# bjg-gh/style_transfer_visualizer

Hardware: AMD Instinct MI355X
Metric: optimization steps/sec at 512² and 1024², 1/2/4/8 MI355X (higher is better)
Workload: dtype bf16; 1 GPU; single 512x512 image per GPU, L-BFGS (max_iter=1, history 100), VGG19 bf16 storage / fp32 accumulate, fp32 Gram, --no-video (BASELINE.json configs[1]); weights: synthetic He-scaled; size=512, images=1, init_method=random, parallelism=replicas x1 (independent images), lbfgs_history_prefill_steps=95, world_size=1

## Files before the change

### style_transfer_visualizer_amd/csrc/gram.hip

```cpp
#include <stdlib.h>

#include "stv_common.h"

namespace {

constexpr int PK = 32;

template <int TS>
struct GramCfg {
  static constexpr int AT = TS / 64;
  static constexpr int PITCH = TS + 4;
  static constexpr int TILE_FLOATS = PK * PITCH;
  static constexpr int STAGE_FLOATS = 2 * TILE_FLOATS;
  static constexpr int LDS_BYTES = 2 * STAGE_FLOATS * 4;
};

inline int gram_tile(int C) { return C <= 64 ? 64 : 128; }

__device__ __forceinline__ uint32_t split_word(float f) {
  const uint32_t hb = (uint32_t)f32_to_bf16(f);
  const float hf = __uint_as_float(hb << 16);
  const float r = __builtin_isfinite(hf) ? f - hf : 0.0f;
  return hb | ((uint32_t)f32_to_bf16(r) << 16);
}

template <typename T, int TS, bool X3 = false>
__device__ __forceinline__ void gram_partial_body(const T* __restrict__ F, float* __restrict__ partials, int N, int C,
                                                  int ksplit, int chunk, int bx, int by) {
  using G = GramCfg<TS>;
  constexpr int kVec = elem_traits<T>::kVec;
  constexpr int VPR = TS / kVec;
  constexpr int VECS = PK * VPR;
  constexpr int ITERS = (VECS + 255) / 256;
  extern __shared__ __attribute__((aligned(16))) char smem_raw[];
  float* smem = reinterpret_cast<float*>(smem_raw);

  const int nt = (C + TS - 1) / TS;
  int ti = 0, rem = bx;
  while (rem >= nt - ti) { rem -= nt - ti; ++ti; }
  const int tj = ti + rem;
  const int i0 = ti * TS, j0 = tj * TS;
  const int ks = by;
  const int p_begin = ks * chunk;
  const int p_end = min(N, p_begin + chunk);

  const int tid = threadIdx.x, lane = tid & 63, wave = tid >> 6;
  const int wi = wave >> 1, wj = wave & 1;
  const int r = lane & 31, h = lane >> 5;

  f32x16 acc[G::AT][G::AT];
#pragma unroll
  for (int a = 0; a < G::AT; ++a)
#pragma unroll
    for (int b = 0; b < G::AT; ++b)
#pragma unroll
      for (int i = 0; i < 16; ++i) acc[a][b][i] = 0.0f;

  u32x4 reg_i[ITERS], reg_j[ITERS];
  const u32x4 zero4 = {0u, 0u, 0u, 0u};
  auto stage_load = [&](int p0) {
#pragma unroll
    for (int it = 0; it < ITERS; ++it) {
      const int v = it * 256 + tid;
      const int p = p0 + v / VPR, cv = (v % VPR) * kVec;
      const bool okp = (v < VECS) && p < p_end;
      reg_i[it] = (okp && i0 + cv < C) ? *reinterpret_cast<const u32x4*>(F + (size_t)p * C + i0 + cv) : zero4;
      reg_j[it] = (okp && j0 + cv < C) ? *reinterpret_cast<const u32x4*>(F + (size_t)p * C + j0 + cv) : zero4;
    }
  };
  auto stage_write = [&](float* buf) {
#pragma unroll
    for (int it = 0; it < ITERS; ++it) {
      const int v = it * 256 + tid;
      if (v < VECS) {
        const int pr = v / VPR, cv = (v % VPR) * kVec;
        float fi[kVec], fj[kVec];
        unpack16<T>(reg_i[it], fi);
        unpack16<T>(reg_j[it], fj);
        if constexpr (X3) {
#pragma unroll
          for (int e = 0; e < kVec; ++e) {
            fi[e] = __uint_as_float(split_word(fi[e]));
            fj[e] = __uint_as_float(split_word(fj[e]));
          }
        }
#pragma unroll
        for (int q = 0; q < kVec / 4; ++q) {
          *reinterpret_cast<f32x4*>(buf + pr * G::PITCH + cv + 4 * q) =
              f32x4{fi[4 * q], fi[4 * q + 1], fi[4 * q + 2], fi[4 * q + 3]};
          *reinterpret_cast<f32x4*>(buf + G::TILE_FLOATS + pr * G::PITCH + cv + 4 * q) =
              f32x4{fj[4 * q], fj[4 * q + 1], fj[4 * q + 2], fj[4 * q + 3]};
        }
      }
    }
  };

  const int nstages = (p_end > p_begin) ? (p_end - p_begin + PK - 1) / PK : 0;
  if (nstages > 0) {
    stage_load(p_begin);
    stage_write(smem);
  }
  __syncthreads();
  for (int s = 0; s < nstages; ++s) {
    float* cur = smem + (s & 1) * G::STAGE_FLOATS;
    float* nxt = smem + ((s + 1) & 1) * G::STAGE_FLOATS;
    const bool more = (s + 1) < nstages;
    if (more) stage_load(p_begin + (s + 1) * PK);
    const float* ai = cur + wi * (G::AT * 32) + r;
    const float* bj = cur + G::TILE_FLOATS + wj * (G::AT * 32) + r;
    if constexpr (X3) {
      auto frag = [&](const float* base, bf16x8v& hi, bf16x8v& lo) {
        uint32_t w[8];
#pragma unroll
        for (int e = 0; e < 8; ++e) w[e] = __float_as_uint(base[(8 * h + e) * G::PITCH]);
        u32x4 vh, vl;
#pragma unroll
        for (int e = 0; e < 4; ++e) {
          vh[e] = __builtin_amdgcn_perm(w[2 * e + 1], w[2 * e], 0x05040100u);
          vl[e] = __builtin_amdgcn_perm(w[2 * e + 1], w[2 * e], 0x07060302u);
        }
        hi = __builtin_bit_cast(bf16x8v, vh);
        lo = __builtin_bit_cast(bf16x8v, vl);
      };
#pragma unroll
      for (int kk = 0; kk < PK / 16; ++kk) {
        bf16x8v ah[G::AT], al[G::AT], bh[G::AT], bl[G::AT];
#pragma unroll
        for (int a = 0; a < G::AT; ++a) frag(ai + kk * 16 * G::PITCH + a * 32, ah[a], al[a]);
#pragma unroll
        for (int b = 0; b < G::AT; ++b) frag(bj + kk * 16 * G::PITCH + b * 32, bh[b], bl[b]);
#pragma unroll
        for (int a = 0; a < G::AT; ++a)
#pragma unroll
          for (int b = 0; b < G::AT; ++b) {
            acc[a][b] = __builtin_amdgcn_mfma_f32_32x32x16_bf16(ah[a], bh[b], acc[a][b], 0, 0, 0);
            acc[a][b] = __builtin_amdgcn_mfma_f32_32x32x16_bf16(ah[a], bl[b], acc[a][b], 0, 0, 0);
            acc[a][b] = __builtin_amdgcn_mfma_f32_32x32x16_bf16(al[a], bh[b], acc[a][b], 0, 0, 0);
          }
      }
    } else
#pragma unroll
    for (int q = 0; q < PK / 2; ++q) {
      float av[G::AT], bv[G::AT];
#pragma unroll
      for (int a = 0; a < G::AT; ++a) av[a] = ai[(2 * q + h) * G::PITCH + a * 32];
#pragma unroll
      for (int b = 0; b < G::AT; ++b) bv[b] = bj[(2 * q + h) * G::PITCH + b * 32];
#pragma unroll
      for (int a = 0; a < G::AT; ++a)
#pragma unroll
        for (int b = 0; b < G::AT; ++b)
          acc[a][b] = __builtin_amdgcn_mfma_f32_32x32x2f32(av[a], bv[b], acc[a][b], 0, 0, 0);
    }
    if (more) stage_write(nxt);
    __syncthreads();
  }

  float* out = partials + (size_t)ks * C * C;
#pragma unroll
  for (int a = 0; a < G::AT; ++a)
#pragma unroll
    for (int b = 0; b < G::AT; ++b)
#pragma unroll
      for (int i = 0; i < 16; ++i) {
        const int row = i0 + wi * (G::AT * 32) + a * 32 + (i & 3) + 8 * (i >> 2) + 4 * h;
        const int col = j0 + wj * (G::AT * 32) + b * 32 + r;
        if (row < C && col < C) out[(size_t)row * C + col] = acc[a][b][i];
      }
}

constexpr int kMaxTaps = 8;
struct PartialMulti {
  int n;
  int block0[kMaxTaps + 1];
  const void* F[kMaxTaps];
  float* partials[kMaxTaps];
  int N[kMaxTaps], C[kMaxTaps], ksplit[kMaxTaps], chunk[kMaxTaps], pairs[kMaxTaps];
};
__device__ __forceinline__ int find_tap(const int* block0, int n, int b) {
  int i = 0;
  while (i + 1 < n && b >= block0[i + 1]) ++i;
  return i;
}

__device__ __forceinline__ void decode_block(int b, int pairs, int ksplit, int& pair, int& ks) {
  pair = b % pairs;
  ks = b / pairs;
}

using PartialSingleFn = void (*)(const void*, float*, int, int, int, int, int);
template <typename T, int TS, bool X3 = false>
__global__ __launch_bounds__(256) void gram_partial_kernel(const void* __restrict__ F, float* __restrict__ partials,
                                                           int N, int C, int ksplit, int chunk, int pairs) {
  int pair, ks;
  decode_block(blockIdx.x, pairs, ksplit, pair, ks);
  gram_partial_body<T, TS, X3>(static_cast<const T*>(F), partials, N, C, ksplit, chunk, pair, ks);
}
template <typename T, int TS, bool X3 = false>
__global__ __launch_bounds__(256) void gram_partial_multi_kernel(PartialMulti m) {
  const int i = find_tap(m.block0, m.n, blockIdx.x);
  const int b = blockIdx.x - m.block0[i];
  int pair, ks;
  decode_block(b, m.pairs[i], m.ksplit[i], pair, ks);
  gram_partial_body<T, TS, X3>(static_cast<const T*>(m.F[i]), m.partials[i], m.N[i], m.C[i], m.ksplit[i], m.chunk[i],
                           pair, ks);
}

typedef __attribute__((ext_vector_type(4))) short s16x4;
typedef __attribute__((address_space(3))) s16x4 lds_s16x4;

#ifndef STV_GRAM_PKB
#define STV_GRAM_PKB 64
#endif
constexpr int PKB = STV_GRAM_PKB;

template <int TS>
struct GramBCfg {
  static constexpr int AT = TS / 64;
  static constexpr int PITCH = TS * 2 + 64;
  static constexpr int TILE_BYTES = PKB * PITCH;
  static constexpr int STAGE_BYTES = 2 * TILE_BYTES;
  static constexpr int LDS_BYTES = 2 * STAGE_BYTES;
};

#ifdef STV_GRAM_STAMPS
__device__ unsigned long long g_gram_stamps[8];
#define GRAM_T() wall_clock64()
#else
#define GRAM_T() 0ull
#endif

template <int TS>
__device__ __forceinline__ void gram_partial_bf16_body(const bf16_t* __restrict__ F, float* __restrict__ partials,
                                                       int N, int C, int ksplit, int chunk, int bx, int by) {
  using G = GramBCfg<TS>;
  constexpr int VPR = TS / 8;
  constexpr int VECS = PKB * VPR;
  constexpr int ITERS = VECS / 256;
  static_assert(VECS % 256 == 0, "whole iterations");
  extern __shared__ __attribute__((aligned(16))) char smem[];

  const int nt = (C + TS - 1) / TS;
  int ti = 0, rem = bx;
  while (rem >= nt - ti) { rem -= nt - ti; ++ti; }
  const int tj = ti + rem;
  const bool same = ti == tj;
  const int i0 = ti * TS, j0 = tj * TS;
  const int ks = by;
  const int p_begin = ks * chunk;
  const int p_end = min(N, p_begin + chunk);

  const int tid = threadIdx.x, lane = tid & 63, wave = tid >> 6;
  const int wi = wave >> 1, wj = wave & 1;
  const int grp = lane >> 4, lam = lane & 15;
  const int tr_lane = ((grp >> 1) * 8 + (lam >> 2)) * G::PITCH + ((grp & 1) * 16 + (lam & 3) * 4) * 2;

  f32x16 acc[G::AT][G::AT];
#pragma unroll
  for (int a = 0; a < G::AT; ++a)
#pragma unroll
    for (int b = 0; b < G::AT; ++b)
#pragma unroll
      for (int i = 0; i < 16; ++i) acc[a][b][i] = 0.0f;

  const __amdgpu_buffer_rsrc_t rs = __builtin_amdgcn_make_buffer_rsrc(
      const_cast<bf16_t*>(F), 0, N * C * 2, 0x00020000);
  const __amdgpu_buffer_rsrc_t rs_null = __builtin_amdgcn_make_buffer_rsrc(const_cast<bf16_t*>(F), 0, 0, 0x00020000);
  constexpr uint32_t kOob = 0x80000000u;
  uint32_t off_i[ITERS], off_j[ITERS];
  int lds_off[ITERS];
#pragma unroll
  for (int it = 0; it < ITERS; ++it) {
    const int v = it * 256 + tid;
    const int pr = v / VPR, cv = (v % VPR) * 8;
    lds_off[it] = pr * G::PITCH + cv * 2;
    off_i[it] = (i0 + cv < C) ? (uint32_t)((pr * C + i0 + cv) * 2) : kOob;
    off_j[it] = (j0 + cv < C) ? (uint32_t)((pr * C + j0 + cv) * 2) : kOob;
  }
  u32x4 reg_i[ITERS], reg_j[ITERS];
  auto stage_load = [&](int p0, bool live) {
    const int rows = min(PKB, p_end - p0);
    const __amdgpu_buffer_rsrc_t r =
        (live && rows > 0) ? __builtin_amdgcn_make_buffer_rsrc(const_cast<bf16_t*>(F) + (size_t)p0 * C, 0,
                                                               rows * C * 2, 0x00020000)
                           : rs_null;
#pragma unroll
    for (int it = 0; it < ITERS; ++it) {
      reg_i[it] = __builtin_amdgcn_raw_buffer_load_b128(r, off_i[it], 0, 0);
      if (!same) reg_j[it] = __builtin_amdgcn_raw_buffer_load_b128(r, off_j[it], 0, 0);
    }
  };
  auto stage_write = [&](char* buf) {
#pragma unroll
    for (int it = 0; it < ITERS; ++it) {
      *reinterpret_cast<u32x4*>(buf + lds_off[it]) = reg_i[it];
      if (!same) *reinterpret_cast<u32x4*>(buf + G::TILE_BYTES + lds_off[it]) = reg_j[it];
    }
  };
  (void)rs;

  const int nstages = (p_end > p_begin) ? (p_end - p_begin + PKB - 1) / PKB : 0;
  unsigned long long tt[6] = {0, 0, 0, 0, 0, 0};
  const unsigned long long t_begin = GRAM_T();
  stage_load(p_begin, nstages > 0);
  stage_write(smem);
  __syncthreads();
  const unsigned long long t_loop = GRAM_T();
  for (int s = 0; s < nstages; ++s) {
    const unsigned long long t0 = GRAM_T();
    char* cur = smem + (s & 1) * G::STAGE_BYTES;
    char* nxt = smem + ((s + 1) & 1) * G::STAGE_BYTES;
    stage_load(p_begin + (s + 1) * PKB, (s + 1) < nstages);
    __builtin_amdgcn_sched_barrier(0);
    const char* ta = cur + tr_lane + (wi * (G::AT * 32)) * 2;
    const char* tb = cur + (same ? 0 : G::TILE_BYTES) + tr_lane + (wj * (G::AT * 32)) * 2;
#pragma unroll
    for (int kk = 0; kk < PKB / 16; ++kk) {
      bf16x8v af[G::AT], bfr[G::AT];
#pragma unroll
      for (int a = 0; a < G::AT; ++a) {
        const char* pa = ta + kk * 16 * G::PITCH + a * 64;
        const s16x4 lo = __builtin_amdgcn_ds_read_tr16_b64_v4i16((lds_s16x4*)(pa));
        const s16x4 hi = __builtin_amdgcn_ds_read_tr16_b64_v4i16((lds_s16x4*)(pa + 4 * G::PITCH));
        typedef __attribute__((ext_vector_type(8))) short s16x8;
        const s16x8 v = {lo[0], lo[1], lo[2], lo[3], hi[0], hi[1], hi[2], hi[3]};
        af[a] = __builtin_bit_cast(bf16x8v, v);
      }
#pragma unroll
      for (int b = 0; b < G::AT; ++b) {
        const char* pb = tb + kk * 16 * G::PITCH + b * 64;
        const s16x4 lo = __builtin_amdgcn_ds_read_tr16_b64_v4i16((lds_s16x4*)(pb));
        const s16x4 hi = __builtin_amdgcn_ds_read_tr16_b64_v4i16((lds_s16x4*)(pb + 4 * G::PITCH));
        typedef __attribute__((ext_vector_type(8))) short s16x8;
        const s16x8 v = {lo[0], lo[1], lo[2], lo[3], hi[0], hi[1], hi[2], hi[3]};
        bfr[b] = __builtin_bit_cast(bf16x8v, v);
      }
#pragma unroll
      for (int a = 0; a < G::AT; ++a)
#pragma unroll
        for (int b = 0; b < G::AT; ++b)
          acc[a][b] = __builtin_amdgcn_mfma_f32_32x32x16_bf16(af[a], bfr[b], acc[a][b], 0, 0, 0);
    }
    __builtin_amdgcn_sched_barrier(0);
#ifdef STV_GRAM_STAMPS
    const unsigned long long t1 = GRAM_T();
    __builtin_amdgcn_s_waitcnt(0x0F70);
    const unsigned long long t2 = GRAM_T();
    stage_write(nxt);
    __builtin_amdgcn_s_waitcnt(0xC07F);
    const unsigned long long t3 = GRAM_T();
    __syncthreads();
    const unsigned long long t4 = GRAM_T();
    tt[0] += t1 - t0; tt[1] += t2 - t1; tt[2] += t3 - t2; tt[3] += t4 - t3;
#else
    stage_write(nxt);
    __syncthreads();
#endif
  }
  const unsigned long long t_end = GRAM_T();

  const int r = lane & 31, h = lane >> 5;
  float* out = partials + (size_t)ks * C * C;
#pragma unroll
  for (int a = 0; a < G::AT; ++a)
#pragma unroll
    for (int b = 0; b < G::AT; ++b)
#pragma unroll
      for (int i = 0; i < 16; ++i) {
        const int row = i0 + wi * (G::AT * 32) + a * 32 + (i & 3) + 8 * (i >> 2) + 4 * h;
        const int col = j0 + wj * (G::AT * 32) + b * 32 + r;
        if (row < C && col < C) out[(size_t)row * C + col] = acc[a][b][i];
      }
#ifdef STV_GRAM_STAMPS
  if (bx == 0 && by == 0 && tid == 0) {
    g_gram_stamps[0] = tt[0]; g_gram_stamps[1] = tt[1]; g_gram_stamps[2] = tt[2]; g_gram_stamps[3] = tt[3];
    g_gram_stamps[4] = t_loop - t_begin; g_gram_stamps[5] = GRAM_T() - t_end; g_gram_stamps[6] = nstages;
  }
#endif
}

template <int TS>
__global__ __launch_bounds__(256) void gram_partial_bf16_kernel(const void* __restrict__ F, float* __restrict__ partials,
                                                                int N, int C, int ksplit, int chunk, int pairs) {
  int pair, ks;
  decode_block(blockIdx.x, pairs, ksplit, pair, ks);
  gram_partial_bf16_body<TS>(static_cast<const bf16_t*>(F), partials, N, C, ksplit, chunk, pair, ks);
}
template <int TS>
__global__ __launch_bounds__(256) void gram_partial_bf16_multi_kernel(PartialMulti m) {
  const int i = find_tap(m.block0, m.n, blockIdx.x);
  const int b = blockIdx.x - m.block0[i];
  int pair, ks;
  decode_block(b, m.pairs[i], m.ksplit[i], pair, ks);
  gram_partial_bf16_body<TS>(static_cast<const bf16_t*>(m.F[i]), m.partials[i], m.N[i], m.C[i], m.ksplit[i],
                             m.chunk[i], pair, ks);
}

__global__ __launch_bounds__(256) void gram_partial_bf16_both_kernel(PartialMulti m128, PartialMulti m64) {
  const int n128 = m128.block0[m128.n];
  int pair, ks;
  if ((int)blockIdx.x < n128) {
    const int i = find_tap(m128.block0, m128.n, blockIdx.x);
    decode_block(blockIdx.x - m128.block0[i], m128.pairs[i], m128.ksplit[i], pair, ks);
    gram_partial_bf16_body<128>(static_cast<const bf16_t*>(m128.F[i]), m128.partials[i], m128.N[i], m128.C[i],
                                m128.ksplit[i], m128.chunk[i], pair, ks);
  } else {
    const int b = (int)blockIdx.x - n128;
    const int i = find_tap(m64.block0, m64.n, b);
    decode_block(b - m64.block0[i], m64.pairs[i], m64.ksplit[i], pair, ks);
    gram_partial_bf16_body<64>(static_cast<const bf16_t*>(m64.F[i]), m64.partials[i], m64.N[i], m64.C[i], m64.ksplit[i],
                               m64.chunk[i], pair, ks);
  }
}

constexpr int FIN_V = 4, FIN_L = 32, FIN_E = FIN_L * FIN_V, FIN_U = 4;
template <typename T, int FIN_S>
__device__ __forceinline__ void gram_finish_body(
    const float* __restrict__ partials, const float* __restrict__ target, float* __restrict__ gram_out,
    float* __restrict__ loss_part, T* __restrict__ sgrad, int C, int TS, int ksplit, float clamp_max,
    float norm, float k_grad, const float* __restrict__ coef_dev, int bx) {
  __shared__ f32x4 red[FIN_S][FIN_L];
  const int le = threadIdx.x % FIN_L;
  const int slice = threadIdx.x / FIN_L;
  const int e = bx * FIN_E + le * FIN_V;
  const int CC = C * C;
  const int i = e / C, j = e - i * C;
  const bool lower = (i / TS) > (j / TS);
  const bool mirror = (i / TS) < (j / TS);
  const f32x4 zero = {0.f, 0.f, 0.f, 0.f};
  f32x4 s = zero;
  if (e < CC && !lower) {
    f32x4 acc[FIN_U];
#pragma unroll
    for (int u = 0; u < FIN_U; ++u) acc[u] = zero;
    const float* src = partials + e;
    int ks = slice;
    for (; ks + (FIN_U - 1) * FIN_S < ksplit; ks += FIN_U * FIN_S) {
#pragma unroll
      for (int u = 0; u < FIN_U; ++u)
        acc[u] += *reinterpret_cast<const f32x4*>(src + (size_t)(ks + u * FIN_S) * CC);
    }
#pragma unroll
    for (int u = 0; u < FIN_U; ++u)
      if (ks + u * FIN_S < ksplit) acc[u] += *reinterpret_cast<const f32x4*>(src + (size_t)(ks + u * FIN_S) * CC);
    s = (acc[0] + acc[1]) + (acc[2] + acc[3]);
  }
  red[slice][le] = s;
  __syncthreads();
  if (slice == 0) {
    float d2 = 0.0f;
    if (e < CC && !lower) {
      f32x4 R = zero;
#pragma unroll
      for (int q = 0; q < FIN_S; ++q) R += red[q][le];
      const float kk = (target && sgrad) ? k_grad * (coef_dev ? *coef_dev : 1.0f) : 0.0f;
      f32x4 Gv, tv = zero;
#pragma unroll
      for (int v = 0; v < FIN_V; ++v) Gv[v] = fminf(R[v], clamp_max) / norm;
      if (gram_out) *reinterpret_cast<f32x4*>(gram_out + e) = Gv;
      if (target) {
        tv = *reinterpret_cast<const f32x4*>(target + e);
#pragma unroll
        for (int v = 0; v < FIN_V; ++v) {
          const float d = Gv[v] - tv[v];
          d2 += d * d;
          if (sgrad) elem_traits<T>::store(sgrad + e + v, (R[v] <= clamp_max) ? kk * d : 0.0f);
        }
      }
      if (mirror) {
#pragma unroll
        for (int v = 0; v < FIN_V; ++v) {
          const int em = (j + v) * C + i;
          if (gram_out) gram_out[em] = Gv[v];
          if (target) {
            const float dm = Gv[v] - target[em];
            d2 += dm * dm;
            if (sgrad) elem_traits<T>::store(sgrad + em, (R[v] <= clamp_max) ? kk * dm : 0.0f);
          }
        }
      }
    }
#pragma unroll
    for (int o = FIN_L / 2; o > 0; o >>= 1) d2 += __shfl_xor(d2, o, FIN_L);
    if (le == 0 && loss_part) loss_part[bx] = d2;
  }
}

struct FinishMulti {
  int n;
  int block0[kMaxTaps + 1];
  const float* partials[kMaxTaps];
  const float* target[kMaxTaps];
  float* gram_out[kMaxTaps];
  float* loss_part[kMaxTaps];
  void* sgrad[kMaxTaps];
  const float* coef_dev[kMaxTaps];
  int C[kMaxTaps], TS[kMaxTaps], ksplit[kMaxTaps];
  float clamp_max[kMaxTaps], norm[kMaxTaps], k_grad[kMaxTaps];
};
template <typename T, int FIN_S>
__global__ __launch_bounds__(FIN_L * FIN_S) void gram_finish_multi_kernel(FinishMulti m) {
  const int i = find_tap(m.block0, m.n, blockIdx.x);
  gram_finish_body<T, FIN_S>(m.partials[i], m.target[i], m.gram_out[i], m.loss_part[i], static_cast<T*>(m.sgrad[i]), m.C[i],
                         m.TS[i], m.ksplit[i], m.clamp_max[i], m.norm[i], m.k_grad[i], m.coef_dev[i],
                         blockIdx.x - m.block0[i]);
}

void add_tap(PartialMulti& m, const void* F, float* partials, int N, int C, int pk) {
  const int nt = ceil_div(C, gram_tile(C)), pairs = nt * (nt + 1) / 2;
  const int ksplit = stv_gram_ksplit(N, C);
  const int k = m.n++;
  m.F[k] = F; m.partials[k] = partials; m.N[k] = N; m.C[k] = C;
  m.ksplit[k] = ksplit; m.chunk[k] = ceil_div(ceil_div(N, ksplit), pk) * pk; m.pairs[k] = pairs;
  m.block0[k + 1] = m.block0[k] + pairs * ksplit;
}

enum { BODY_F32 = STV_F32, BODY_BF16 = STV_BF16, BODY_X3 = STV_BF16X3, BODY_BF16_WIDE };
static_assert(BODY_F32 == 0 && BODY_BF16 == 1 && BODY_X3 == 2, "the table below is indexed by dtype code");
struct PartialKernel {
  PartialSingleFn single;
  void (*multi)(PartialMulti);
  int lds;
};
#define STV_GENERIC(T, X3, TS) {gram_partial_kernel<T, TS, X3>, gram_partial_multi_kernel<T, TS, X3>, GramCfg<TS>::LDS_BYTES}
const PartialKernel kPartialKernels[4][2] = {
    {STV_GENERIC(float, false, 64), STV_GENERIC(float, false, 128)},
    {{gram_partial_bf16_kernel<64>, gram_partial_bf16_multi_kernel<64>, GramBCfg<64>::LDS_BYTES},
     {gram_partial_bf16_kernel<128>, gram_partial_bf16_multi_kernel<128>, GramBCfg<128>::LDS_BYTES}},
    {STV_GENERIC(float, true, 64), STV_GENERIC(float, true, 128)},
    {{gram_partial_kernel<bf16_t, 64>, nullptr, GramCfg<64>::LDS_BYTES}, {gram_partial_kernel<bf16_t, 128>, nullptr, GramCfg<128>::LDS_BYTES}},
};
#undef STV_GENERIC
constexpr int kBothLds = GramBCfg<128>::LDS_BYTES > GramBCfg<64>::LDS_BYTES ? GramBCfg<128>::LDS_BYTES : GramBCfg<64>::LDS_BYTES;

inline int pixels_per_stage(int body) { return body == BODY_BF16 ? PKB : PK; }

int launch_partial(int body, int TS, const PartialMulti& m, hipStream_t st) {
  const PartialKernel& k = kPartialKernels[body][TS == 128];
  const dim3 grid(m.block0[m.n]), block(256);
  if (m.n == 1) {
    if (stv_set_max_lds(reinterpret_cast<const void*>(k.single), k.lds) != STV_OK) return STV_ERR_LAUNCH;
    hipLaunchKernelGGL(k.single, grid, block, k.lds, st, m.F[0], m.partials[0], m.N[0], m.C[0], m.ksplit[0], m.chunk[0], m.pairs[0]);
  } else {
    if (!k.multi) return STV_ERR_ARG;
    if (stv_set_max_lds(reinterpret_cast<const void*>(k.multi), k.lds) != STV_OK) return STV_ERR_LAUNCH;
    hipLaunchKernelGGL(k.multi, grid, block, k.lds, st, m);
  }
  STV_CHECK_LAUNCH();
  return STV_OK;
}

void add_finish_tap(FinishMulti& f, const stv_gram_tap_t& t) {
  const int k = f.n++;
  f.partials[k] = t.partials; f.target[k] = t.target; f.gram_out[k] = t.gram_out; f.loss_part[k] = t.loss_part;
  f.sgrad[k] = t.sgrad; f.coef_dev[k] = t.coef_dev; f.C[k] = t.channels; f.TS[k] = gram_tile(t.channels);
  f.ksplit[k] = stv_gram_ksplit(t.n_pixels, t.channels);
  f.clamp_max[k] = t.clamp_max; f.norm[k] = t.norm;
  f.k_grad[k] = t.coef * 4.0f / ((float)t.channels * (float)t.channels * t.norm);
  f.block0[k + 1] = f.block0[k] + stv_gram_loss_parts(t.channels);
}

template <typename T, int S>
int launch_finish_as(const FinishMulti& f, hipStream_t st) {
  hipLaunchKernelGGL((gram_finish_multi_kernel<T, S>), dim3(f.block0[f.n]), dim3(FIN_L * S), 0, st, f);
  STV_CHECK_LAUNCH();
  return STV_OK;
}
int launch_finish(const FinishMulti& f, bool bf16_seed, bool deep, hipStream_t st) {
  if (bf16_seed) return deep ? launch_finish_as<bf16_t, 32>(f, st) : launch_finish_as<bf16_t, 8>(f, st);
  return deep ? launch_finish_as<float, 32>(f, st) : launch_finish_as<float, 8>(f, st);
}

}

extern "C" int stv_gram_ksplit(int n_pixels, int channels) {
  const int TS = gram_tile(channels);
  const int nt = ceil_div(channels, TS);
  const int pairs = nt * (nt + 1) / 2;
  static const int wg_max = getenv("STV_GRAM_WGS") ? atoi(getenv("STV_GRAM_WGS")) : 512;
  static const int wg_min = getenv("STV_GRAM_WGS_MIN") ? atoi(getenv("STV_GRAM_WGS_MIN")) : 128;
  const int lo = ceil_div(wg_min, pairs), hi = (wg_max / pairs) > 0 ? wg_max / pairs : 1;
  static const int kdiv = getenv("STV_GRAM_KDIV") ? atoi(getenv("STV_GRAM_KDIV")) : 8;
  int ks = n_pixels / (kdiv * channels);
  if (ks < lo) ks = lo;
  if (ks > hi) ks = hi;
  const int max_ks = ceil_div(n_pixels, 64);
  if (ks > max_ks) ks = max_ks;
  if (ks < 1) ks = 1;
  return ks;
}

extern "C" size_t stv_gram_partials_bytes(int n_pixels, int channels) {
  return (size_t)stv_gram_ksplit(n_pixels, channels) * channels * channels * sizeof(float);
}

extern "C" int stv_gram_loss_parts(int channels) { return ceil_div(channels * channels, FIN_E); }

extern "C" int stv_gram_partial(const void* F, float* partials, int n_pixels, int C, int dtype,
                                void* stream) {
  if (!F || !partials || n_pixels <= 0 || C <= 0) return STV_ERR_ARG;
  if (dtype != STV_F32 && dtype != STV_BF16 && dtype != STV_BF16X3) return STV_ERR_ARG;
  const bool bf16 = dtype == STV_BF16;
  if (C % (bf16 ? 8 : 4)) return STV_ERR_ARG;
  const bool huge = (size_t)n_pixels * C * (bf16 ? 2 : 4) >= ((size_t)1 << 31);
  if (dtype == STV_BF16X3 && huge) return STV_ERR_ARG;
  const int body = (bf16 && huge) ? BODY_BF16_WIDE : dtype;
  PartialMulti m{};
  add_tap(m, F, partials, n_pixels, C, pixels_per_stage(body));
  return launch_partial(body, gram_tile(C), m, static_cast<hipStream_t>(stream));
}

extern "C" int stv_gram_finish(const float* partials, const float* target, float* gram_out,
                               float* loss_part, void* sgrad, int n_pixels, int C, float clamp_max,
                               float norm, float coef, const float* coef_dev, int dtype, void* stream) {
  if (!partials || n_pixels <= 0 || C <= 0 || norm <= 0.0f) return STV_ERR_ARG;
  if (dtype != STV_F32 && dtype != STV_BF16) return STV_ERR_ARG;
  FinishMulti f{};
  add_finish_tap(f, stv_gram_tap_t{nullptr, const_cast<float*>(partials), target, gram_out, loss_part, sgrad, coef_dev,
                                   n_pixels, C, clamp_max, norm, coef});
  return launch_finish(f, dtype == STV_BF16, f.ksplit[0] >= 128, static_cast<hipStream_t>(stream));
}

extern "C" int stv_gram_multi(const stv_gram_tap_t* taps, int n_taps, int dtype, void* stream) {
  if (!taps || n_taps <= 0 || n_taps > kMaxTaps) return STV_ERR_ARG;
  if (dtype != STV_F32 && dtype != STV_BF16 && dtype != STV_BF16X3) return STV_ERR_ARG;
  hipStream_t st = static_cast<hipStream_t>(stream);
  const bool x3 = dtype == STV_BF16X3;
  const int vec = dtype == STV_BF16 ? 8 : 4;
  for (int i = 0; i < n_taps; ++i) {
    const stv_gram_tap_t& t = taps[i];
    if (!t.partials || t.n_pixels <= 0 || t.channels <= 0 || t.channels % vec || t.norm <= 0.0f) return STV_ERR_ARG;
    if (dtype == STV_BF16 && (size_t)t.n_pixels * t.channels * 2 >= ((size_t)1 << 31)) return STV_ERR_ARG;
    if (x3 && t.F && (size_t)t.n_pixels * t.channels * 4 >= ((size_t)1 << 31)) return STV_ERR_ARG;
  }
  PartialMulti by_tile[2] = {};
  for (int i = 0; i < n_taps; ++i) {
    const stv_gram_tap_t& t = taps[i];
    if (!t.F) continue;
    add_tap(by_tile[gram_tile(t.channels) == 128], t.F, t.partials, t.n_pixels, t.channels, pixels_per_stage(dtype));
  }
  const PartialMulti& m64 = by_tile[0];
  const PartialMulti& m128 = by_tile[1];
  if (dtype == STV_BF16 && m64.n && m128.n) {
    if (stv_set_max_lds(reinterpret_cast<const void*>(&gram_partial_bf16_both_kernel), kBothLds) != STV_OK) return STV_ERR_LAUNCH;
    hipLaunchKernelGGL(gram_partial_bf16_both_kernel, dim3(m128.block0[m128.n] + m64.block0[m64.n]), dim3(256), kBothLds, st,
                       m128, m64);
    STV_CHECK_LAUNCH();
  } else {
    for (int TS : {64, 128}) {
      const PartialMulti& m = by_tile[TS == 128];
      if (!m.n) continue;
      if (const int rc = launch_partial(dtype, TS, m, st)) return rc;
    }
  }
  FinishMulti f{};
  for (int i = 0; i < n_taps; ++i) add_finish_tap(f, taps[i]);
  return launch_finish(f, dtype == STV_BF16, false, st);
}

#ifdef STV_GRAM_STAMPS
extern "C" int stv_debug_gram_stamps(unsigned long long* out8) {
  return hipMemcpyFromSymbol(out8, HIP_SYMBOL(g_gram_stamps), sizeof(g_gram_stamps)) == hipSuccess ? 0 : 1;
}
#endif
```

Measured before the change: 1248 steps/s.

## Split gram finish into short and long paths with batched partial loads

```diff
diff --git a/style_transfer_visualizer_amd/csrc/gram.hip b/style_transfer_visualizer_amd/csrc/gram.hip
--- a/style_transfer_visualizer_amd/csrc/gram.hip
+++ b/style_transfer_visualizer_amd/csrc/gram.hip
@@ -414,74 +414,196 @@
 }
 
 constexpr int FIN_V = 4, FIN_L = 32, FIN_E = FIN_L * FIN_V, FIN_U = 4;
+constexpr int FIN_HOIST = 4;
+
+inline int finish_blocks(int C, int ksplit, int fin_s) {
+  const int parts = ceil_div(C * C, FIN_E);
+  return ksplit <= FIN_U * fin_s ? ceil_div(parts, fin_s) : parts;
+}
+
+struct FinishQuad {
+  int e, i, j;
+  bool live, mirror;
+};
+__device__ __forceinline__ FinishQuad finish_quad(int e, int C, int TS) {
+  FinishQuad q;
+  q.e = e;
+  q.i = e / C;
+  q.j = e - q.i * C;
+  q.live = e < C * C && (q.i / TS) <= (q.j / TS);
+  q.mirror = (q.i / TS) < (q.j / TS);
+  return q;
+}
+
+struct FinishTargets {
+  f32x4 own;
+  float mir[FIN_V];
+  float coef;
+};
+__device__ __forceinline__ FinishTargets finish_request_targets(const float* __restrict__ target,
+                                                                const float* __restrict__ coef_dev, const FinishQuad& q, int C) {
+  FinishTargets t;
+  t.coef = coef_dev ? *coef_dev : 1.0f;
+  t.own = f32x4{0.f, 0.f, 0.f, 0.f};
+#pragma unroll
+  for (int v = 0; v < FIN_V; ++v) t.mir[v] = 0.0f;
+  if (target) {
+    t.own = *reinterpret_cast<const f32x4*>(target + q.e);
+    if (q.mirror) {
+#pragma unroll
+      for (int v = 0; v < FIN_V; ++v) t.mir[v] = target[(q.j + v) * C + q.i];
+    }
+  }
+  return t;
+}
+
+template <typename T>
+__device__ __forceinline__ float finish_store(const f32x4 R, const FinishTargets& t, const FinishQuad& q,
+                                              const float* __restrict__ target, float* __restrict__ gram_out,
+                                              T* __restrict__ sgrad, int C, float clamp_max, float norm, float k_grad) {
+  float d2 = 0.0f;
+  const float kk = (target && sgrad) ? k_grad * t.coef : 0.0f;
+  f32x4 Gv;
+#pragma unroll
+  for (int v = 0; v < FIN_V; ++v) Gv[v] = fminf(R[v], clamp_max) / norm;
+  if (gram_out) *reinterpret_cast<f32x4*>(gram_out + q.e) = Gv;
+  if (target) {
+    float d[FIN_V];
+#pragma unroll
+    for (int v = 0; v < FIN_V; ++v) d[v] = Gv[v] - t.own[v];
+    static_assert(FIN_V == 4, "the chain below");
+    d2 = fmaf(d[3], d[3], fmaf(d[2], d[2], fmaf(d[0], d[0], d[1] * d[1])));
+    if (sgrad) {
+#pragma unroll
+      for (int v = 0; v < FIN_V; ++v) elem_traits<T>::store(sgrad + q.e + v, (R[v] <= clamp_max) ? kk * d[v] : 0.0f);
+    }
+  }
+  if (q.mirror) {
+#pragma unroll
+    for (int v = 0; v < FIN_V; ++v) {
+      const int em = (q.j + v) * C + q.i;
+      if (gram_out) gram_out[em] = Gv[v];
+      if (target) {
+        const float dm = Gv[v] - t.mir[v];
+        d2 = fmaf(dm, dm, d2);
+        if (sgrad) elem_traits<T>::store(sgrad + em, (R[v] <= clamp_max) ? kk * dm : 0.0f);
+      }
+    }
+  }
+  return d2;
+}
+
+__device__ __forceinline__ float finish_group_sum(float d2) {
+#pragma unroll
+  for (int o = FIN_L / 2; o > 0; o >>= 1) d2 += __shfl_xor(d2, o, FIN_L);
+  return d2;
+}
+
 template <typename T, int FIN_S>
-__device__ __forceinline__ void gram_finish_body(
+__device__ __forceinline__ void gram_finish_short(
+    const float* __restrict__ partials, const float* __restrict__ target, float* __restrict__ gram_out,
+    float* __restrict__ loss_part, T* __restrict__ sgrad, int C, int TS, int ksplit, float clamp_max,
+    float norm, float k_grad, const float* __restrict__ coef_dev, int bx) {
+  constexpr int B = FIN_S <= 8 ? FIN_S : 4;
+  static_assert(FIN_S % B == 0, "whole batches");
+  const int le = threadIdx.x % FIN_L;
+  const int grp = bx * FIN_S + threadIdx.x / FIN_L;
+  const int CC = C * C;
+  const FinishQuad q = finish_quad(grp * FIN_E + le * FIN_V, C, TS);
+  const f32x4 zero = {0.f, 0.f, 0.f, 0.f};
+  float d2 = 0.0f;
+  if (q.live) {
+    const float* src = partials + q.e;
+    f32x4 val[B][FIN_U];
+    auto request = [&](int q0) {
+#pragma unroll
+      for (int b = 0; b < B; ++b)
+#pragma unroll
+        for (int u = 0; u < FIN_U; ++u) {
+          const int ks = q0 + b + u * FIN_S;
+          val[b][u] = ks < ksplit ? *reinterpret_cast<const f32x4*>(src + (size_t)ks * CC) : zero;
+        }
+    };
+    const FinishTargets t = finish_request_targets(target, coef_dev, q, C);
+    f32x4 R = zero;
+#pragma unroll 1
+    for (int q0 = 0; q0 < FIN_S; q0 += B) {
+      request(q0);
+#pragma unroll
+      for (int b = 0; b < B; ++b)
+#pragma unroll
+        for (int u = 0; u < FIN_U; ++u) asm volatile("" : "+v"(val[b][u]));
+#pragma unroll
+      for (int b = 0; b < B; ++b) {
+        f32x4 acc[FIN_U];
+#pragma unroll
+        for (int u = 0; u < FIN_U; ++u) acc[u] = zero + val[b][u];
+        R += (acc[0] + acc[1]) + (acc[2] + acc[3]);
+      }
+    }
+    d2 = finish_store<T>(R, t, q, target, gram_out, sgrad, C, clamp_max, norm, k_grad);
+  }
+  d2 = finish_group_sum(d2);
+  if (le == 0 && loss_part && grp * FIN_E < CC) loss_part[grp] = d2;
+}
+
+template <typename T, int FIN_S>
+__device__ __forceinline__ void gram_finish_long(
     const float* __restrict__ partials, const float* __restrict__ target, float* __restrict__ gram_out,
     float* __restrict__ loss_part, T* __restrict__ sgrad, int C, int TS, int ksplit, float clamp_max,
     float norm, float k_grad, const float* __restrict__ coef_dev, int bx) {
   __shared__ f32x4 red[FIN_S][FIN_L];
   const int le = threadIdx.x % FIN_L;
   const int slice = threadIdx.x / FIN_L;
-  const int e = bx * FIN_E + le * FIN_V;
   const int CC = C * C;
-  const int i = e / C, j = e - i * C;
-  const bool lower = (i / TS) > (j / TS);
-  const bool mirror = (i / TS) < (j / TS);
+  const FinishQuad q = finish_quad(bx * FIN_E + le * FIN_V, C, TS);
   const f32x4 zero = {0.f, 0.f, 0.f, 0.f};
   f32x4 s = zero;
-  if (e < CC && !lower) {
+  FinishTargets t{};
+  if (slice == 0 && q.live) t = finish_request_targets(target, coef_dev, q, C);
+  if (q.live) {
     f32x4 acc[FIN_U];
 #pragma unroll
     for (int u = 0; u < FIN_U; ++u) acc[u] = zero;
-    const float* src = partials + e;
+    const float* src = partials + q.e;
+    f32x4 val[FIN_HOIST][FIN_U];
     int ks = slice;
-    for (; ks + (FIN_U - 1) * FIN_S < ksplit; ks += FIN_U * FIN_S) {
+    for (; ks + (FIN_HOIST * FIN_U - 1) * FIN_S < ksplit; ks += FIN_HOIST * FIN_U * FIN_S) {
+#pragma unroll
+      for (int h = 0; h < FIN_HOIST; ++h)
+#pragma unroll
+        for (int u = 0; u < FIN_U; ++u)
+          val[h][u] = *reinterpret_cast<const f32x4*>(src + (size_t)(ks + (h * FIN_U + u) * FIN_S) * CC);
+#pragma unroll
+      for (int h = 0; h < FIN_HOIST; ++h)
+#pragma unroll
+        for (int u = 0; u < FIN_U; ++u) acc[u] += val[h][u];
+    }
+#pragma unroll
+    for (int h = 0; h < FIN_HOIST; ++h)
+#pragma unroll
+      for (int u = 0; u < FIN_U; ++u) {
+        const int k = ks + (h * FIN_U + u) * FIN_S;
+        if (k < ksplit) val[h][u] = *reinterpret_cast<const f32x4*>(src + (size_t)k * CC);
+      }
+#pragma unroll
+    for (int h = 0; h < FIN_HOIST; ++h)
 #pragma unroll
       for (int u = 0; u < FIN_U; ++u)
-        acc[u] += *reinterpret_cast<const f32x4*>(src + (size_t)(ks + u * FIN_S) * CC);
-    }
-#pragma unroll
-    for (int u = 0; u < FIN_U; ++u)
-      if (ks + u * FIN_S < ksplit) acc[u] += *reinterpret_cast<const f32x4*>(src + (size_t)(ks + u * FIN_S) * CC);
+        if (ks + (h * FIN_U + u) * FIN_S < ksplit) acc[u] += val[h][u];
     s = (acc[0] + acc[1]) + (acc[2] + acc[3]);
   }
   red[slice][le] = s;
   __syncthreads();
   if (slice == 0) {
     float d2 = 0.0f;
-    if (e < CC && !lower) {
+    if (q.live) {
       f32x4 R = zero;
 #pragma unroll
-      for (int q = 0; q < FIN_S; ++q) R += red[q][le];
-      const float kk = (target && sgrad) ? k_grad * (coef_dev ? *coef_dev : 1.0f) : 0.0f;
-      f32x4 Gv, tv = zero;
-#pragma unroll
-      for (int v = 0; v < FIN_V; ++v) Gv[v] = fminf(R[v], clamp_max) / norm;
-      if (gram_out) *reinterpret_cast<f32x4*>(gram_out + e) = Gv;
-      if (target) {
-        tv = *reinterpret_cast<const f32x4*>(target + e);
-#pragma unroll
-        for (int v = 0; v < FIN_V; ++v) {
-          const float d = Gv[v] - tv[v];
-          d2 += d * d;
-          if (sgrad) elem_traits<T>::store(sgrad + e + v, (R[v] <= clamp_max) ? kk * d : 0.0f);
-        }
-      }
-      if (mirror) {
-#pragma unroll
-        for (int v = 0; v < FIN_V; ++v) {
-          const int em = (j + v) * C + i;
-          if (gram_out) gram_out[em] = Gv[v];
-          if (target) {
-            const float dm = Gv[v] - target[em];
-            d2 += dm * dm;
-            if (sgrad) elem_traits<T>::store(sgrad + em, (R[v] <= clamp_max) ? kk * dm : 0.0f);
-          }
-        }
-      }
-    }
-#pragma unroll
-    for (int o = FIN_L / 2; o > 0; o >>= 1) d2 += __shfl_xor(d2, o, FIN_L);
+      for (int k = 0; k < FIN_S; ++k) R += red[k][le];
+      d2 = finish_store<T>(R, t, q, target, gram_out, sgrad, C, clamp_max, norm, k_grad);
+    }
+    d2 = finish_group_sum(d2);
     if (le == 0 && loss_part) loss_part[bx] = d2;
   }
 }
@@ -501,9 +623,13 @@
 template <typename T, int FIN_S>
 __global__ __launch_bounds__(FIN_L * FIN_S) void gram_finish_multi_kernel(FinishMulti m) {
   const int i = find_tap(m.block0, m.n, blockIdx.x);
-  gram_finish_body<T, FIN_S>(m.partials[i], m.target[i], m.gram_out[i], m.loss_part[i], static_cast<T*>(m.sgrad[i]), m.C[i],
-                         m.TS[i], m.ksplit[i], m.clamp_max[i], m.norm[i], m.k_grad[i], m.coef_dev[i],
-                         blockIdx.x - m.block0[i]);
+  const int bx = blockIdx.x - m.block0[i];
+  if (m.ksplit[i] <= FIN_U * FIN_S)
+    gram_finish_short<T, FIN_S>(m.partials[i], m.target[i], m.gram_out[i], m.loss_part[i], static_cast<T*>(m.sgrad[i]),
+                                m.C[i], m.TS[i], m.ksplit[i], m.clamp_max[i], m.norm[i], m.k_grad[i], m.coef_dev[i], bx);
+  else
+    gram_finish_long<T, FIN_S>(m.partials[i], m.target[i], m.gram_out[i], m.loss_part[i], static_cast<T*>(m.sgrad[i]),
+                               m.C[i], m.TS[i], m.ksplit[i], m.clamp_max[i], m.norm[i], m.k_grad[i], m.coef_dev[i], bx);
 }
 
 void add_tap(PartialMulti& m, const void* F, float* partials, int N, int C, int pk) {
@@ -550,14 +676,14 @@
   return STV_OK;
 }
 
-void add_finish_tap(FinishMulti& f, const stv_gram_tap_t& t) {
+void add_finish_tap(FinishMulti& f, const stv_gram_tap_t& t, int fin_s) {
   const int k = f.n++;
   f.partials[k] = t.partials; f.target[k] = t.target; f.gram_out[k] = t.gram_out; f.loss_part[k] = t.loss_part;
   f.sgrad[k] = t.sgrad; f.coef_dev[k] = t.coef_dev; f.C[k] = t.channels; f.TS[k] = gram_tile(t.channels);
   f.ksplit[k] = stv_gram_ksplit(t.n_pixels, t.channels);
   f.clamp_max[k] = t.clamp_max; f.norm[k] = t.norm;
   f.k_grad[k] = t.coef * 4.0f / ((float)t.channels * (float)t.channels * t.norm);
-  f.block0[k + 1] = f.block0[k] + stv_gram_loss_parts(t.channels);
+  f.block0[k + 1] = f.block0[k] + finish_blocks(t.channels, f.ksplit[k], fin_s);
 }
 
 template <typename T, int S>
@@ -566,9 +692,10 @@
   STV_CHECK_LAUNCH();
   return STV_OK;
 }
+constexpr int kFinS = 8, kFinSDeep = 32;
 int launch_finish(const FinishMulti& f, bool bf16_seed, bool deep, hipStream_t st) {
-  if (bf16_seed) return deep ? launch_finish_as<bf16_t, 32>(f, st) : launch_finish_as<bf16_t, 8>(f, st);
-  return deep ? launch_finish_as<float, 32>(f, st) : launch_finish_as<float, 8>(f, st);
+  if (bf16_seed) return deep ? launch_finish_as<bf16_t, kFinSDeep>(f, st) : launch_finish_as<bf16_t, kFinS>(f, st);
+  return deep ? launch_finish_as<float, kFinSDeep>(f, st) : launch_finish_as<float, kFinS>(f, st);
 }
 
 }
@@ -616,9 +743,10 @@
   if (!partials || n_pixels <= 0 || C <= 0 || norm <= 0.0f) return STV_ERR_ARG;
   if (dtype != STV_F32 && dtype != STV_BF16) return STV_ERR_ARG;
   FinishMulti f{};
+  const bool deep = stv_gram_ksplit(n_pixels, C) >= 128;
   add_finish_tap(f, stv_gram_tap_t{nullptr, const_cast<float*>(partials), target, gram_out, loss_part, sgrad, coef_dev,
-                                   n_pixels, C, clamp_max, norm, coef});
-  return launch_finish(f, dtype == STV_BF16, f.ksplit[0] >= 128, static_cast<hipStream_t>(stream));
+                                   n_pixels, C, clamp_max, norm, coef}, deep ? kFinSDeep : kFinS);
+  return launch_finish(f, dtype == STV_BF16, deep, static_cast<hipStream_t>(stream));
 }
 
 extern "C" int stv_gram_multi(const stv_gram_tap_t* taps, int n_taps, int dtype, void* stream) {
@@ -654,7 +782,7 @@
     }
   }
   FinishMulti f{};
-  for (int i = 0; i < n_taps; ++i) add_finish_tap(f, taps[i]);
+  for (int i = 0; i < n_taps; ++i) add_finish_tap(f, taps[i], kFinS);
   return launch_finish(f, dtype == STV_BF16, false, st);
 }
 
```

After: 1241 steps/s, median of 2. No clear change (-0.6%).
